# JuliaLinearAlgebra/RecursiveFactorization.jl

Measured on AMD Instinct MI355X. Metric: LU GFLOP/s (2n^3/3) on NxN Float64, 1/2/4/8 MI355X; ||PA-LU||/||A||, higher is better.
Workload: dtype f64; 1 GPU; lu!(A, ipiv) of a dense uniform[0,1) 16384x16384 Float64 matrix, partial pivoting, column-major in HBM; n=16384, pivot=True, blocksize=0, layout=single GPU

## Files before the change

recursivefactorization.jl_amd/csrc/gemm_tile.hpp:

```cpp
#pragma once

#include <stdlib.h>

#include <algorithm>
#include <type_traits>

#include "rflu_internal.hpp"

namespace rflu {

template <typename T>
struct Mfma;

template <>
struct Mfma<double> {
    typedef double acc_t __attribute__((ext_vector_type(4)));
    static __device__ __forceinline__ acc_t run(double a, double b, acc_t c) {
        return __builtin_amdgcn_mfma_f64_16x16x4f64(a, b, c, 0, 0, 0);
    }
    static constexpr bool HAS_NEG = true;
    static __device__ __forceinline__ acc_t run_neg(double a, double b, acc_t c) {
        return __builtin_amdgcn_mfma_f64_16x16x4f64(a, b, c, 0, 0, 1);
    }
    static __device__ __forceinline__ int crow(int lane, int r) { return (lane >> 4) + 4 * r; }
};

template <>
struct Mfma<float> {
    typedef float acc_t __attribute__((ext_vector_type(4)));
    static __device__ __forceinline__ acc_t run(float a, float b, acc_t c) {
        return __builtin_amdgcn_mfma_f32_16x16x4f32(a, b, c, 0, 0, 0);
    }
    static constexpr bool HAS_NEG = false;
    static __device__ __forceinline__ acc_t run_neg(float a, float b, acc_t c) { return run(-a, b, c); }
    static __device__ __forceinline__ int crow(int lane, int r) { return 4 * (lane >> 4) + r; }
};

constexpr int G_BM = 128, G_BN = 128, G_BK = 16;
constexpr int G_SA = G_BK + 1;
constexpr int G_SB = G_BN + 16;
constexpr int G_STAGE = G_BM * G_SA + G_BK * G_SB;
#ifndef RFLU_GEMM_GROUP_M
#define RFLU_GEMM_GROUP_M 8
#endif
constexpr int G_GROUP_M = RFLU_GEMM_GROUP_M;
#ifndef RFLU_GEMM_SSTORE_AT
#define RFLU_GEMM_SSTORE_AT 4
#endif
#ifndef RFLU_GEMM_PRIO
#define RFLU_GEMM_PRIO 1
#endif
constexpr int G_PRIO = RFLU_GEMM_PRIO;
constexpr int G_SSTORE_AT = RFLU_GEMM_SSTORE_AT;
#ifndef RFLU_GEMM_CSPLIT
#define RFLU_GEMM_CSPLIT 3
#endif
constexpr int G_CSPLIT = RFLU_GEMM_CSPLIT;

template <typename T>
struct GemmArgs {
    int M, N, K;
    const T* A;
    int64_t lda;
    const T* B;
    int64_t ldb;
    T* C;
    int64_t ldc;
    int tiles_m, tiles_n;
    int vec_ok;
    int flags;
    int na_tiles_n;
    unsigned long long* sig_flag;
    unsigned long long sig_val;
    unsigned* sig_cnt;
#if defined(RFLU_GEMM_TRACE)
    unsigned long long* stamps;
#endif
};

#if defined(RFLU_GEMM_TRACE)
static unsigned long long* g_gemm_stamps = nullptr;
extern "C" void rflu_debug_gemm_stamps(unsigned long long* p) { g_gemm_stamps = p; }
#define GEMM_STAMP(k)                                                                                                  \
    do {                                                                                                               \
        if (g.stamps && tid == 0) g.stamps[(size_t)blockIdx.x * 8 + (k)] = wall_clock64(); \
    } while (0)
#else
#define GEMM_STAMP(k) do { } while (0)
#endif

template <typename T, bool C_FIRST, bool INTERIOR>
__device__ __forceinline__ void gemm_tile(const GemmArgs<T>& g, T* smem, const int m0, const int n0)
{
    typedef typename Mfma<T>::acc_t acc_t;
    constexpr int VW = 16 / (int)sizeof(T);
    typedef T vec_t __attribute__((ext_vector_type(VW)));
    constexpr bool NEGMOD = C_FIRST && Mfma<T>::HAS_NEG;
    constexpr bool NEGACC = C_FIRST && !Mfma<T>::HAS_NEG;
    constexpr bool SPLITC = INTERIOR && sizeof(T) == 8;
    const int tid = threadIdx.x;
    const int lane = tid & 63;
    const int wave = tid >> 6;
    const int wr = wave >> 1, wc = wave & 1;

    const int a_row = tid >> 1, a_kb = (tid & 1) * 8;
    const int b_k = tid >> 4, b_jb = (tid & 15) * 8;
    const T* Ap = g.A + (int64_t)(m0 + a_row) * g.lda + a_kb;
    const T* Bp = g.B + (int64_t)b_k * g.ldb + n0 + b_jb;
    const bool a_row_ok = (m0 + a_row) < g.M;
    const bool full_mn = INTERIOR || (g.vec_ok && (m0 + G_BM <= g.M) && (n0 + G_BN <= g.N));

#if defined(RFLU_GEMM_TRACE)
    if (g.stamps && tid == 0) {
        unsigned hwid, xcc;
        asm volatile("s_getreg_b32 %0, hwreg(HW_REG_HW_ID)" : "=s"(hwid));
        asm volatile("s_getreg_b32 %0, hwreg(HW_REG_XCC_ID)" : "=s"(xcc));
        g.stamps[(size_t)blockIdx.x * 8 + 4] = ((unsigned long long)xcc << 32) | hwid;
    }
#endif
    GEMM_STAMP(0);
    T ra[8], rb[8];

    auto gload = [&](int k0) {
        if (INTERIOR || (full_mn && (k0 + G_BK <= g.K))) {
#pragma unroll
            for (int v = 0; v < 8 / VW; ++v) {
                vec_t x = *reinterpret_cast<const vec_t*>(Ap + k0 + v * VW);
                vec_t y = *reinterpret_cast<const vec_t*>(Bp + (int64_t)k0 * g.ldb + v * VW);
#pragma unroll
                for (int e = 0; e < VW; ++e) {
                    ra[v * VW + e] = x[e];
                    rb[v * VW + e] = y[e];
                }
            }
        } else {
            const bool bk_ok = (k0 + b_k) < g.K;
#pragma unroll
            for (int e = 0; e < 8; ++e) {
                ra[e] = (a_row_ok && (k0 + a_kb + e) < g.K) ? Ap[k0 + e] : T(0);
                rb[e] = (bk_ok && (n0 + b_jb + e) < g.N) ? Bp[(int64_t)k0 * g.ldb + e] : T(0);
            }
        }
    };
    auto sstore = [&](int stage) {
        T* As = smem + stage * G_STAGE;
        T* Bs = As + G_BM * G_SA;
#pragma unroll
        for (int e = 0; e < 8; ++e) {
            As[a_row * G_SA + a_kb + e] = ra[e];
            Bs[b_k * G_SB + b_jb + (b_jb >> 4) + e] = rb[e];
        }
    };

    const bool ntc = (g.flags & 2) != 0;
    const bool wt = (g.flags & 4) != 0;
    gload(0);
    acc_t acc[4][4];
    auto load_c = [&](int i_lo, int i_hi) {
#pragma unroll
        for (int i = 0; i < 4; ++i) {
            if (i < i_lo || i >= i_hi) continue;
#pragma unroll
            for (int r = 0; r < 4; ++r) {
                const int row = m0 + wr * 64 + i * 16 + Mfma<T>::crow(lane, r);
                const T* crow_p = g.C + (int64_t)row * g.ldc + n0 + wc * 64 + (lane & 15);
#pragma unroll
                for (int j = 0; j < 4; ++j) {
                    const int col = n0 + wc * 64 + j * 16 + (lane & 15);
                    T cv = T(0);
#ifdef RFLU_GEMM_EXP_NOCLOAD
                    if (false)
#else
                    if (C_FIRST && (full_mn || (row < g.M && col < g.N)))
#endif
                        cv = ntc ? __builtin_nontemporal_load(crow_p + j * 16) : crow_p[j * 16];
                    acc[i][j][r] = (NEGACC && !SPLITC) ? -cv : cv;
                }
            }
        }
    };
    const int nk = (g.K + G_BK - 1) / G_BK;
    load_c(0, SPLITC ? G_CSPLIT : 4);
#if defined(RFLU_GEMM_TRACE) && RFLU_GEMM_TRACE == 2
    GEMM_STAMP(6);
    sstore(0);
    asm volatile("s_waitcnt lgkmcnt(0)" ::: "memory");
    GEMM_STAMP(7);
    __syncthreads();
#else
    sstore(0);
    __syncthreads();
#endif
    if (SPLITC) load_c(G_CSPLIT, 4);
    GEMM_STAMP(1);
#if defined(RFLU_GEMM_TRACE) && RFLU_GEMM_TRACE != 2
    if (g.stamps && tid == 0) g.stamps[(size_t)blockIdx.x * 8 + 6] = clock64();
#endif

    const int a_frag = (wr * 64 + (lane & 15)) * G_SA + (lane >> 4);
    const int b_frag = (lane >> 4) * G_SB + wc * 68 + (lane & 15);

    auto slab = [&](int kt, bool more, auto first) {
        const int cur = kt & 1;
#ifndef RFLU_GEMM_EXP_NOLOAD
        if (more) gload((kt + 1) * G_BK);
#endif
        const T* As = smem + cur * G_STAGE;
        const T* Bs = As + G_BM * G_SA;
        if (G_PRIO) __builtin_amdgcn_s_setprio(G_PRIO);
#pragma unroll
        for (int kk = 0; kk < G_BK / 4; ++kk) {
            if (kk == G_SSTORE_AT && more) sstore(cur ^ 1);
            T a[4], b[4];
#pragma unroll
            for (int t = 0; t < 4; ++t) {
                a[t] = As[a_frag + t * 16 * G_SA + kk * 4];
                b[t] = Bs[b_frag + kk * 4 * G_SB + t * 17];
            }
#pragma unroll
            for (int i = 0; i < 4; ++i) {
                if (NEGACC && SPLITC && decltype(first)::value && kk == 0) {
#pragma unroll
                    for (int j = 0; j < 4; ++j) acc[i][j] = -acc[i][j];
                }
#pragma unroll
                for (int j = 0; j < 4; ++j) acc[i][j] = NEGMOD ? Mfma<T>::run_neg(a[i], b[j], acc[i][j]) : Mfma<T>::run(a[i], b[j], acc[i][j]);
            }
        }
        if (G_PRIO) __builtin_amdgcn_s_setprio(0);
        if (G_SSTORE_AT >= G_BK / 4 && more) sstore(cur ^ 1);
#ifndef RFLU_GEMM_EXP_NOBARRIER
        __syncthreads();
#endif
    };
    if (SPLITC) {
        slab(0, true, std::true_type{});
        for (int kt = 1; kt + 1 < nk; ++kt) slab(kt, true, std::false_type{});
        slab(nk - 1, false, std::false_type{});
    } else {
        for (int kt = 0; kt < nk; ++kt) slab(kt, kt + 1 < nk, std::false_type{});
    }

    GEMM_STAMP(2);
#if defined(RFLU_GEMM_TRACE) && RFLU_GEMM_TRACE != 2
    if (g.stamps && tid == 0) g.stamps[(size_t)blockIdx.x * 8 + 7] = clock64();
#endif
#pragma unroll
    for (int i = 0; i < 4; ++i) {
#pragma unroll
        for (int r = 0; r < 4; ++r) {
            const int row = m0 + wr * 64 + i * 16 + Mfma<T>::crow(lane, r);
            if (full_mn || row < g.M) {
                T* crow_p = g.C + (int64_t)row * g.ldc + n0 + wc * 64 + (lane & 15);
#pragma unroll
                for (int j = 0; j < 4; ++j) {
                    const int col = n0 + wc * 64 + j * 16 + (lane & 15);
                    if (full_mn || col < g.N) {
                        if (C_FIRST) {
                            const T out = NEGACC ? -acc[i][j][r] : acc[i][j][r];
                            if (wt) __hip_atomic_store(crow_p + j * 16, out, __ATOMIC_RELAXED, __HIP_MEMORY_SCOPE_AGENT);
                            else if (ntc) __builtin_nontemporal_store(out, crow_p + j * 16);
                            else crow_p[j * 16] = out;
                        } else {
                            crow_p[j * 16] = crow_p[j * 16] - acc[i][j][r];
                        }
                    }
                }
            }
        }
    }
    GEMM_STAMP(3);
#if defined(RFLU_GEMM_TRACE)
    if (g.stamps) { __builtin_amdgcn_s_waitcnt(0x0F70); GEMM_STAMP(5); }
#endif
}

}
```

Baseline: 41960 GFLOP/s.

## Software-pipeline interior GEMM tile with register double-buffered fragments and interleaved fills

Adds a pipelined main loop for interior f64 GEMM tiles. It prefetches global data two K-slabs ahead, double-buffers LDS fragment reads in registers, and interleaves the shared-memory stores and global loads piecewise between MFMA groups. Sched barriers enforce the placement, and the block barrier is moved ahead of the last few MFMAs so they can overlap it. The aim is to hide LDS-store, global-load and barrier latency behind matrix-core work. In exchange it raises register pressure and removes the older store-position and negation options, which may affect the float path.

```diff
diff --git a/recursivefactorization.jl_amd/csrc/gemm_tile.hpp b/recursivefactorization.jl_amd/csrc/gemm_tile.hpp
--- a/recursivefactorization.jl_amd/csrc/gemm_tile.hpp
+++ b/recursivefactorization.jl_amd/csrc/gemm_tile.hpp
@@ -44,18 +44,19 @@
 #define RFLU_GEMM_GROUP_M 8
 #endif
 constexpr int G_GROUP_M = RFLU_GEMM_GROUP_M;
-#ifndef RFLU_GEMM_SSTORE_AT
-#define RFLU_GEMM_SSTORE_AT 4
-#endif
 #ifndef RFLU_GEMM_PRIO
 #define RFLU_GEMM_PRIO 1
 #endif
 constexpr int G_PRIO = RFLU_GEMM_PRIO;
-constexpr int G_SSTORE_AT = RFLU_GEMM_SSTORE_AT;
 #ifndef RFLU_GEMM_CSPLIT
 #define RFLU_GEMM_CSPLIT 3
 #endif
 constexpr int G_CSPLIT = RFLU_GEMM_CSPLIT;
+#ifndef RFLU_GEMM_PIPE
+#define RFLU_GEMM_PIPE 1
+#endif
+constexpr int G_PIPE = RFLU_GEMM_PIPE;
+constexpr int G_PIPE_POST = 2;
 
 template <typename T>
 struct GemmArgs {
@@ -98,6 +99,8 @@
     constexpr bool NEGMOD = C_FIRST && Mfma<T>::HAS_NEG;
     constexpr bool NEGACC = C_FIRST && !Mfma<T>::HAS_NEG;
     constexpr bool SPLITC = INTERIOR && sizeof(T) == 8;
+    constexpr bool PIPE = INTERIOR && ((G_PIPE & (sizeof(T) == 8 ? 1 : 2)) != 0);
+    constexpr int NV = 8 / VW;
     const int tid = threadIdx.x;
     const int lane = tid & 63;
     const int wave = tid >> 6;
@@ -141,6 +144,13 @@
                 rb[e] = (bk_ok && (n0 + b_jb + e) < g.N) ? Bp[(int64_t)k0 * g.ldb + e] : T(0);
             }
         }
+    };
+    auto gload_piece = [&](int k0, int p) {
+        const int v = p % NV;
+        const vec_t x = p < NV ? *reinterpret_cast<const vec_t*>(Ap + k0 + v * VW)
+                               : *reinterpret_cast<const vec_t*>(Bp + (int64_t)k0 * g.ldb + v * VW);
+#pragma unroll
+        for (int e = 0; e < VW; ++e) (p < NV ? ra : rb)[v * VW + e] = x[e];
     };
     auto sstore = [&](int stage) {
         T* As = smem + stage * G_STAGE;
@@ -184,11 +194,19 @@
 #if defined(RFLU_GEMM_TRACE) && RFLU_GEMM_TRACE == 2
     GEMM_STAMP(6);
     sstore(0);
+    if (PIPE) {
+#pragma unroll
+        for (int p = 0; p < 2 * NV; ++p) gload_piece(G_BK, p);
+    }
     asm volatile("s_waitcnt lgkmcnt(0)" ::: "memory");
     GEMM_STAMP(7);
     __syncthreads();
 #else
     sstore(0);
+    if (PIPE) {
+#pragma unroll
+        for (int p = 0; p < 2 * NV; ++p) gload_piece(G_BK, p);
+    }
     __syncthreads();
 #endif
     if (SPLITC) load_c(G_CSPLIT, 4);
@@ -200,17 +218,14 @@
     const int a_frag = (wr * 64 + (lane & 15)) * G_SA + (lane >> 4);
     const int b_frag = (lane >> 4) * G_SB + wc * 68 + (lane & 15);
 
-    auto slab = [&](int kt, bool more, auto first) {
+    auto slab = [&](int kt, bool more) {
         const int cur = kt & 1;
-#ifndef RFLU_GEMM_EXP_NOLOAD
         if (more) gload((kt + 1) * G_BK);
-#endif
         const T* As = smem + cur * G_STAGE;
         const T* Bs = As + G_BM * G_SA;
         if (G_PRIO) __builtin_amdgcn_s_setprio(G_PRIO);
 #pragma unroll
         for (int kk = 0; kk < G_BK / 4; ++kk) {
-            if (kk == G_SSTORE_AT && more) sstore(cur ^ 1);
             T a[4], b[4];
 #pragma unroll
             for (int t = 0; t < 4; ++t) {
@@ -219,26 +234,92 @@
             }
 #pragma unroll
             for (int i = 0; i < 4; ++i) {
-                if (NEGACC && SPLITC && decltype(first)::value && kk == 0) {
-#pragma unroll
-                    for (int j = 0; j < 4; ++j) acc[i][j] = -acc[i][j];
-                }
 #pragma unroll
                 for (int j = 0; j < 4; ++j) acc[i][j] = NEGMOD ? Mfma<T>::run_neg(a[i], b[j], acc[i][j]) : Mfma<T>::run(a[i], b[j], acc[i][j]);
             }
         }
         if (G_PRIO) __builtin_amdgcn_s_setprio(0);
-        if (G_SSTORE_AT >= G_BK / 4 && more) sstore(cur ^ 1);
-#ifndef RFLU_GEMM_EXP_NOBARRIER
+        if (more) sstore(cur ^ 1);
         __syncthreads();
-#endif
-    };
-    if (SPLITC) {
-        slab(0, true, std::true_type{});
-        for (int kt = 1; kt + 1 < nk; ++kt) slab(kt, true, std::false_type{});
-        slab(nk - 1, false, std::false_type{});
+    };
+
+    constexpr int PIECE_EVERY = 8 / (2 * NV);
+    constexpr int FILL_AT = 16 - G_PIPE_POST - 8;
+    T fa[2][4], fb[2][4];
+    auto fread = [&](int set, int stage, int kk) {
+        const T* As = smem + stage * G_STAGE;
+        const T* Bs = As + G_BM * G_SA;
+#pragma unroll
+        for (int t = 0; t < 4; ++t) {
+            fa[set][t] = As[a_frag + t * 16 * G_SA + kk * 4];
+            fb[set][t] = Bs[b_frag + kk * 4 * G_SB + t * 17];
+        }
+    };
+    auto mfmas = [&](int set, int lo, int hi) {
+#pragma unroll
+        for (int u = 0; u < 16; ++u) {
+            if (u < lo || u >= hi) continue;
+            const int i = u >> 2, j = u & 3;
+            acc[i][j] = NEGMOD ? Mfma<T>::run_neg(fa[set][i], fb[set][j], acc[i][j]) : Mfma<T>::run(fa[set][i], fb[set][j], acc[i][j]);
+        }
+    };
+    auto fill_piece = [&](int stage, int p) {
+        T* As = smem + stage * G_STAGE;
+        T* Bs = As + G_BM * G_SA;
+        const int v = p % NV;
+#pragma unroll
+        for (int e = 0; e < VW; ++e) {
+            if (p < NV) As[a_row * G_SA + a_kb + v * VW + e] = ra[v * VW + e];
+            else Bs[b_k * G_SB + b_jb + (b_jb >> 4) + v * VW + e] = rb[v * VW + e];
+        }
+    };
+    auto slab_p = [&](int kt, int kload, auto fill_t, auto load_t) {
+        constexpr bool FILL = decltype(fill_t)::value, LOAD = decltype(load_t)::value;
+        const int cur = kt & 1;
+        if (G_PRIO) __builtin_amdgcn_s_setprio(G_PRIO);
+#pragma unroll
+        for (int kk = 0; kk < G_BK / 4; ++kk) {
+            const int set = kk & 1;
+            if (kk + 1 < G_BK / 4) {
+                fread(set ^ 1, cur, kk + 1);
+                __builtin_amdgcn_sched_barrier(0);
+            }
+            if (kk + 1 < G_BK / 4 || !FILL) {
+                mfmas(set, 0, 16);
+                continue;
+            }
+            mfmas(set, 0, FILL_AT);
+#pragma unroll
+            for (int p = 0; p < 2 * NV; ++p) {
+                __builtin_amdgcn_sched_barrier(0);
+                fill_piece(cur ^ 1, p);
+                if (LOAD) gload_piece(kload * G_BK, p);
+                __builtin_amdgcn_sched_barrier(0);
+                mfmas(set, FILL_AT + p * PIECE_EVERY, FILL_AT + (p + 1) * PIECE_EVERY);
+            }
+            __builtin_amdgcn_sched_barrier(0);
+            if (G_PRIO) __builtin_amdgcn_s_setprio(0);
+            __syncthreads();
+            if (G_PRIO) __builtin_amdgcn_s_setprio(G_PRIO);
+            fread(0, cur ^ 1, 0);
+            __builtin_amdgcn_sched_barrier(0);
+            mfmas(set, 16 - G_PIPE_POST, 16);
+        }
+        if (!FILL) {
+            if (G_PRIO) __builtin_amdgcn_s_setprio(0);
+            __syncthreads();
+        }
+    };
+    if (PIPE) {
+        const std::true_type yes{};
+        const std::false_type no{};
+        fread(0, 0, 0);
+        slab_p(0, min(2, nk - 1), yes, yes);
+        for (int kt = 1; kt + 2 < nk; ++kt) slab_p(kt, kt + 2, yes, yes);
+        if (nk > 2) slab_p(nk - 2, 0, yes, no);
+        slab_p(nk - 1, 0, no, no);
     } else {
-        for (int kt = 0; kt < nk; ++kt) slab(kt, kt + 1 < nk, std::false_type{});
+        for (int kt = 0; kt < nk; ++kt) slab(kt, kt + 1 < nk);
     }
 
     GEMM_STAMP(2);
```

After: 41540 GFLOP/s. 1.0% lower.
